# hsp-iit/roft

Measured on AMD Instinct MI355X. Metric: tracker frames/sec per object (640x480) + ADD-S vs CPU ref, higher is better.
Workload: dtype f64; 1 GPU; BASELINE config #4: 640x480, CV_32FC2 flow grid 1, 64 objects in total, 64 per GPU (sharded by object, no data-path collective; result rows all-gathered over RCCL at N > 1), masks+poses at 5 fps with 6-frame delay, flow-aided masks, re-sync and outlier rejection on, frames submitted in batches of at most 8; objects_per_gpu=64, objects_total=64, width=640, height=480, batch_frames=8, ranks=1, backend=nccl

## Files before the change

roft_amd/csrc/k_ukf.hip:

```cpp
#include "roft_device.h"

#pragma clang fp contract(fast)

namespace roft {

#ifdef ROFT_UKF_PROFILE
#define TICK(L, i) do { __syncthreads(); if (threadIdx.x == 0) { long long _t = clock64(); (L).dbg[i] += _t - (L).t0; (L).t0 = _t; } } while (0)
#else
#define TICK(L, i) do {} while (0)
#endif

constexpr int kUkfThreads = 256;

__device__ __forceinline__ void wave_sync()
{
    __builtin_amdgcn_fence(__ATOMIC_RELEASE, "wavefront");
    __builtin_amdgcn_wave_barrier();
    __builtin_amdgcn_fence(__ATOMIC_ACQUIRE, "wavefront");
}

__device__ __forceinline__ void quat_mul(const double a[4], const double b[4], double o[4])
{
    const double w = a[0] * b[0] - a[1] * b[1] - a[2] * b[2] - a[3] * b[3];
    const double x = a[0] * b[1] + a[1] * b[0] + a[2] * b[3] - a[3] * b[2];
    const double y = a[0] * b[2] - a[1] * b[3] + a[2] * b[0] + a[3] * b[1];
    const double z = a[0] * b[3] + a[1] * b[2] - a[2] * b[1] + a[3] * b[0];
    o[0] = w; o[1] = x; o[2] = y; o[3] = z;
}

__device__ __forceinline__ void half_angle(double n, double& sin_over_n, double& c)
{
    const double h = 0.5 * n;
    if (h < 0.25) {
        const double x = h * h;
        const double sinc = 1.0 + x * (-1.0 / 6.0 + x * (1.0 / 120.0 + x * (-1.0 / 5040.0 + x * (1.0 / 362880.0 +
                            x * (-1.0 / 39916800.0 + x * (1.0 / 6227020800.0))))));
        c = 1.0 + x * (-0.5 + x * (1.0 / 24.0 + x * (-1.0 / 720.0 + x * (1.0 / 40320.0 + x * (-1.0 / 3628800.0 +
            x * (1.0 / 479001600.0 + x * (-1.0 / 87178291200.0)))))));
        sin_over_n = 0.5 * sinc;
    } else {
        sin_over_n = sin(h) / n;
        c = cos(h);
    }
}

__device__ __forceinline__ void quat_boxplus(const double q[4], const double r[3], double o[4])
{
    const double n2 = r[0] * r[0] + r[1] * r[1] + r[2] * r[2];
    double s, c;
    if (n2 < 0.25) {
        const double x = 0.25 * n2;
        s = 0.5 * (1.0 + x * (-1.0 / 6.0 + x * (1.0 / 120.0 + x * (-1.0 / 5040.0 + x * (1.0 / 362880.0 +
                   x * (-1.0 / 39916800.0 + x * (1.0 / 6227020800.0)))))));
        c = 1.0 + x * (-0.5 + x * (1.0 / 24.0 + x * (-1.0 / 720.0 + x * (1.0 / 40320.0 + x * (-1.0 / 3628800.0 +
            x * (1.0 / 479001600.0 + x * (-1.0 / 87178291200.0)))))));
    } else {
        half_angle(sqrt(n2), s, c);
    }
    const double qr[4] = {c, s * r[0], s * r[1], s * r[2]};
    quat_mul(qr, q, o);
}

__device__ __forceinline__ double fast_rcp(double d);

__device__ __forceinline__ void quat_diff(const double a[4], const double b[4], double o[3])
{
    const double bc[4] = {b[0], -b[1], -b[2], -b[3]};
    double p[4];
    quat_mul(a, bc, p);
    const double n2 = p[1] * p[1] + p[2] * p[2] + p[3] * p[3];
    const double sgn = (p[0] < 0.0) ? -1.0 : 1.0;
    double k;
    const double ip0 = fast_rcp(fabs(p[0]));
    const double t2 = n2 * (ip0 * ip0);
    if (t2 <= 0.01) {
        const double at = 1.0 + t2 * (-1.0 / 3.0 + t2 * (1.0 / 5.0 + t2 * (-1.0 / 7.0 + t2 * (1.0 / 9.0 + t2 * (-1.0 / 11.0 +
                          t2 * (1.0 / 13.0 + t2 * (-1.0 / 15.0 + t2 * (1.0 / 17.0))))))));
        k = sgn * 2.0 * at * ip0;
    } else {
        const double n = sqrt(n2);
        if (n == 0.0) { o[0] = o[1] = o[2] = 0.0; return; }
        k = sgn * 2.0 * atan2(n, fabs(p[0])) / n;
    }
    o[0] = k * p[1]; o[1] = k * p[2]; o[2] = k * p[3];
}

constexpr int kCols = 50;

struct UkfTab {
    unsigned jtab[11 * 36 * 2];
    unsigned short tri12[78], tri6[26];
};
static_assert(sizeof(UkfTab) % 16 == 0, "copied in 16-byte words");
constexpr int kUkfTabWords = sizeof(UkfTab) / 16;

struct UkfLds {
    alignas(16) UkfTab tab;
    double P[144];
    double V[144];
    double wP[12];
    double S[144];
    double cs[2][6][2];
    double Q[100];
    double VQ[100];
    double wQ[10];
    double rc[12], rs[12];
    int rp[12], rq[12];
    double mean[13];
    double cov[144];
    double Y[13 * kCols];
    double D[12 * kCols];
    double X[12 * kCols];
    double ymean[13];
    double M4[16], V4[16], w4[4];
    double Py[144], Pxy[144], K[144], KPy[144];
    double aug[12 * 24];
    double innov[12], Kin[12];
    double par[24];
    double meas[13];
    double red[4];
    int flag;
    int twist_timeout;
    long long t0;
    long long dbg[32];
};

__device__ __forceinline__ double fast_rcp(double d)
{
    double x = __builtin_amdgcn_rcp(d);
    x = fma(fma(-d, x, 1.0), x, x);
    x = fma(fma(-d, x, 1.0), x, x);
    return x;
}

__device__ __forceinline__ double fast_rsqrt(double d)
{
    double y = __builtin_amdgcn_rsq(d);
    const double h = 0.5 * d;
    y = fma(y, fma(-h * y, y, 0.5), y);
    y = fma(y, fma(-h * y, y, 0.5), y);
    return y;
}

__device__ __forceinline__ void schur_rotation(double app, double aqq, double apq, double& c, double& s)
{
    const double a = aqq - app, b = 2.0 * apq;
    const int e = __builtin_amdgcn_frexp_exp(fmax(fabs(a), fabs(b)));
    const float af = fabsf((float)ldexp(a, -e)), bf = fabsf((float)ldexp(b, -e));
    const float h2 = af * af + bf * bf;
    const float hyp = h2 * __builtin_amdgcn_rsqf(h2);
    const float tf = bf * __builtin_amdgcn_rcpf(af + hyp);
    const double t = ((a >= 0.0) == (b >= 0.0) || a == 0.0) ? (double)tf : -(double)tf;
    const double x = fma(t, t, 1.0);
    double y = (double)__builtin_amdgcn_rsqf((float)x);
    const double hx = 0.5 * x;
    y = fma(y, fma(-hx * y, y, 0.5), y);
    y = fma(y, fma(-hx * y, y, 0.5), y);
    c = y;
    s = t * y;
}

#ifndef ROFT_JACOBI_TOL
#define ROFT_JACOBI_TOL 1e-6
#endif
constexpr double kJacobiTol = ROFT_JACOBI_TOL;

__host__ __device__ __forceinline__ constexpr void jacobi_pair(int n, int round, int i, int& p, int& q)
{
    if (i == 0) { p = n - 1; q = round; }
    else {
        p = round + i; if (p >= n - 1) p -= n - 1;
        q = round - i; if (q < 0) q += n - 1;
    }
    if (p > q) { const int t = p; p = q; q = t; }
}

__device__ __noinline__ void jacobi_wave(double* A, double* V, int n, UkfLds& L)
{
    const int lane = threadIdx.x;
    for (int i = lane; i < n * n; i += 64) V[i] = ((i / n) == (i % n)) ? 1.0 : 0.0;
    wave_sync();
    const int half = n / 2;
    const bool active = lane < half * half;
    const int ba = active ? lane / half : 0, bb = active ? lane % half : 0;
    for (int sweep = 0; sweep < 40; ++sweep) {
        double off = 0.0, dg = 0.0;
        for (int i = lane; i < n * n; i += 64) {
            const int r = i / n, cidx = i % n;
            const double v = A[i];
            if (r == cidx) dg += v * v; else if (r < cidx) off += v * v;
        }
        for (int o = 32; o > 0; o >>= 1) { off += __shfl_xor(off, o, 64); dg += __shfl_xor(dg, o, 64); }
        if (off <= kJacobiTol * kJacobiTol * dg || off == 0.0) break;
        for (int round = 0; round < n - 1; ++round) {
            int pa, qa, pb, qb;
            jacobi_pair(n, round, ba, pa, qa);
            jacobi_pair(n, round, bb, pb, qb);
            double a00 = 0, a01 = 0, a10 = 0, a11 = 0, v00 = 0, v01 = 0, v10 = 0, v11 = 0;
            if (active) {
                a00 = A[pa * n + pb]; a01 = A[pa * n + qb]; a10 = A[qa * n + pb]; a11 = A[qa * n + qb];
                v00 = V[pa * n + pb]; v01 = V[pa * n + qb]; v10 = V[qa * n + pb]; v11 = V[qa * n + qb];
            }
            double c = 1.0, s = 0.0;
            if (active && ba == bb && a01 != 0.0) schur_rotation(a00, a11, a01, c, s);
            const double ca = __shfl(c, ba * half + ba, 64), sa = __shfl(s, ba * half + ba, 64);
            const double cb = __shfl(c, bb * half + bb, 64), sb = __shfl(s, bb * half + bb, 64);
            if (active) {
                double b00 = cb * a00 - sb * a01, b01 = sb * a00 + cb * a01;
                double b10 = cb * a10 - sb * a11, b11 = sb * a10 + cb * a11;
                double c00 = ca * b00 - sa * b10, c10 = sa * b00 + ca * b10;
                double c01 = ca * b01 - sa * b11, c11 = sa * b01 + ca * b11;
                if (ba == bb) { c01 = c10 = 0.5 * (c01 + c10); }
                A[pa * n + pb] = c00; A[pa * n + qb] = c01; A[qa * n + pb] = c10; A[qa * n + qb] = c11;
                V[pa * n + pb] = cb * v00 - sb * v01; V[pa * n + qb] = sb * v00 + cb * v01;
                V[qa * n + pb] = cb * v10 - sb * v11; V[qa * n + qb] = sb * v10 + cb * v11;
            }
            wave_sync();
        }
    }
    wave_sync();
}

constexpr UkfTab make_ukf_tab()
{
    UkfTab t{};
    for (int i = 0; i < 11 * 36; ++i) {
        const int round = i / 36, l = i % 36;
        int pa = 0, qa = 0, pb = 0, qb = 0;
        jacobi_pair(12, round, l / 6, pa, qa);
        jacobi_pair(12, round, l % 6, pb, qb);
        t.jtab[2 * i] = (unsigned)(pa * 12 + pb) | ((unsigned)(pa * 12 + qb) << 16);
        t.jtab[2 * i + 1] = (unsigned)(qa * 12 + pb) | ((unsigned)(qa * 12 + qb) << 16);
    }
    int e = 0;
    for (int i = 0; i < 12; ++i)
        for (int j = i; j < 12; ++j) t.tri12[e++] = (unsigned short)((i << 8) | j);
    e = 0;
    for (int i = 0; i < 6; ++i)
        for (int j = i; j < 6; ++j) t.tri6[e++] = (unsigned short)((i << 8) | j);
    return t;
}
alignas(16) __device__ const UkfTab g_ukf_tab = make_ukf_tab();

__device__ __noinline__ void jacobi12(double* A, double* V, UkfLds& L)
{
    const int tid = threadIdx.x, wave = tid >> 6, lane = tid & 63;
    for (int i = tid; i < 144; i += kUkfThreads) V[i] = ((i / 12) == (i % 12)) ? 1.0 : 0.0;
    __syncthreads();
    const bool act = lane < 36 && wave < 2;
    const int ba = act ? lane / 6 : 0, bb = act ? lane % 6 : 0;
    double* M = (wave == 0) ? A : V;
    for (int sweep = 0; sweep < 40; ++sweep) {
        if (wave == 0) {
            double off = 0.0, dg = 0.0;
            for (int i = lane; i < 144; i += 64) {
                const int r = i / 12, cidx = i % 12;
                const double v = A[i];
                if (r == cidx) dg += v * v; else if (r < cidx) off += v * v;
            }
            for (int o = 32; o > 0; o >>= 1) { off += __shfl_xor(off, o, 64); dg += __shfl_xor(dg, o, 64); }
            if (lane == 0) L.flag = (off <= kJacobiTol * kJacobiTol * dg || off == 0.0) ? 1 : 0;
        }
        __syncthreads();
        if (L.flag) break;
#ifdef ROFT_UKF_PROFILE
        if (tid == 0) L.dbg[16] += 1;
#endif
        for (int round = 0; round < 11; ++round) {
            int o00 = 0, o01 = 0, o10 = 0, o11 = 0;
            double x00 = 0, x01 = 0, x10 = 0, x11 = 0;
            if (act) {
                const unsigned pkx = L.tab.jtab[2 * (round * 36 + lane)], pky = L.tab.jtab[2 * (round * 36 + lane) + 1];
                o00 = pkx & 0xFFFF; o01 = pkx >> 16; o10 = pky & 0xFFFF; o11 = pky >> 16;
                x00 = M[o00]; x01 = M[o01]; x10 = M[o10]; x11 = M[o11];
                if (wave == 0 && ba == bb) {
                    double c = 1.0, s = 0.0;
                    if (x01 != 0.0) schur_rotation(x00, x11, x01, c, s);
// ... 310 lines not shown
        if (tid < 144) {
            const int i = tid / 12, j = tid % 12;
            double s = 0.0;
            for (int k = 0; k < 12; ++k) s += L.cov[i * 12 + k] * V0[k * 12 + j];
            T[tid] = s;
        }
        __syncthreads();
        if (tid < 144) {
            const int r = tid / 12, c = tid % 12;
            const int i = r < c ? r : c, j = r < c ? c : r;
            double s = 0.0;
            for (int k = 0; k < 12; ++k) s += V0[k * 12 + i] * T[k * 12 + j];
            L.P[tid] = s;
        }
        __syncthreads();
        jacobi12(L.P, L.V, L);
        if (tid < 144) {
            const int i = tid / 12, j = tid % 12;
            double s = 0.0;
            for (int k = 0; k < 12; ++k) s += V0[i * 12 + k] * L.V[k * 12 + j];
            T[tid] = s;
        }
        Vfull = T;
    } else {
        if (tid < 144) L.P[tid] = L.cov[tid];
        __syncthreads();
        jacobi12(L.P, L.V, L);
    }
    double inv_ss = 0.0, m1 = 0.0;
    if (tid < 144) {
        const int i = tid / 12, j = tid % 12;
        const double si = sqrt(fabs(L.P[i * 13])), sj = sqrt(fabs(L.P[j * 13]));
        inv_ss = (si + sj > 0.0) ? fast_rcp(si + sj) : 0.0;
        if (i == j) m1 = si;
        else m1 = 0.5 * (L.P[i * 12 + j] + L.P[j * 12 + i]) * inv_ss;
        M[tid] = (i == j) ? 0.0 : m1;
    }
    __syncthreads();
    if (tid < 144) {
        const int i = tid / 12, j = tid % 12;
        double x1sq = 0.0;
        for (int k = 0; k < 12; ++k) x1sq += M[i * 12 + k] * M[k * 12 + j];
        m1 -= x1sq * inv_ss;
    }
    __syncthreads();
    if (tid < 144) M[tid] = m1;
    __syncthreads();
    if (tid < 144) {
        const int i = tid / 12, j = tid % 12;
        double acc = 0.0;
        for (int k = 0; k < 12; ++k) acc += Vfull[i * 12 + k] * M[k * 12 + j];
        L.S[tid] = acc;
        if (warm) warm[tid] = Vfull[tid];
    }
    if (tid < 12) L.wP[tid] = L.P[tid * 13];
    if (warm && tid == 0) *warm_age = use ? age + 1 : 1;
    __syncthreads();
}

__device__ __noinline__ bool cholesky_state_sqrt(UkfLds& L, bool for_correction, double T, double guard_rot, double guard_bil)
{
    if (!(guard_rot > 0.0)) return false;
    const double th = fmax(L.cov[9 * 13], fmax(L.cov[10 * 13], L.cov[11 * 13]));
    const double wv = fmax(L.cov[3 * 13], fmax(L.cov[4 * 13], L.cov[5 * 13]));
    const double xx = fmax(L.cov[6 * 13], fmax(L.cov[7 * 13], L.cov[8 * 13]));
    const int ok_corr = (int)(th <= guard_rot) & (int)(wv * xx <= guard_bil), ok_pred = (int)(th + T * T * wv <= guard_rot);
    const bool ok = __builtin_amdgcn_readfirstlane(for_correction ? ok_corr : ok_pred) != 0;
#ifdef ROFT_UKF_PROFILE
    if (threadIdx.x == 0 && for_correction) { L.dbg[20] = (long long)(th * 1e9); L.dbg[21] = (long long)(wv * 1e9); L.dbg[22] = (long long)(xx * 1e9); }
#endif
    if (!ok) return false;
    return cholesky_rows<12>(L.cov, L.S, L.rc, L);
}

__device__ void ukf_predict(UkfLds& L, const ObjParams& prm, double T, const UtTable& ut, double* warm,
                            int* warm_age, double chol_guard)
{
    const int lane = threadIdx.x;
    const int n = 21;
    const UtW& w = ut_lookup(ut, n);
    const double sc = w.sc;
    constexpr int kPredCols = 25;
    const double wm0 = w.wm0 + 18.0 * w.wi, wc0 = w.wc0 + 18.0 * w.wi;

    if (prm.q_override) {
        for (int i = lane; i < 100; i += kUkfThreads) L.Q[i] = 0.0;
        __syncthreads();
        for (int i = lane; i < 81; i += kUkfThreads) L.Q[(i / 9) * 10 + (i % 9)] = prm.q_override[i];
    } else if (lane >= 192 && lane < 195) {
        const int i = lane - 192;
        const double psd = L.par[3 + i];
        L.Q[i * 10 + i] = psd * T;
        L.Q[(6 + i) * 10 + (6 + i)] = psd * (T * T * T / 3.0);
        L.Q[i * 10 + (6 + i)] = L.Q[(6 + i) * 10 + i] = psd * (T * T / 2.0);
        L.Q[(3 + i) * 10 + (3 + i)] = L.par[i];
    }
    TICK(L, 1);
    if (!cholesky_state_sqrt(L, false, T, chol_guard, 0.0)) decompose_state_cov(L, warm, warm_age);
    TICK(L, 2);

    if (lane < kPredCols) {
        double d[12], dn[12];
        sigma_perturbation(lane, 0, sc, false, 0.0, L, d, dn);
        double v[3], wv[3], x[3], q[4];
        for (int i = 0; i < 3; ++i) {
            v[i] = L.mean[i] + d[i];
            wv[i] = L.mean[3 + i] + d[3 + i];
            x[i] = L.mean[6 + i] + d[6 + i];
        }
        quat_boxplus(L.mean + 9, d + 9, q);
        for (int i = 0; i < 3; ++i) {
            L.Y[i * kCols + lane] = v[i];
            L.Y[(3 + i) * kCols + lane] = wv[i];
            L.Y[(6 + i) * kCols + lane] = x[i] + v[i] * T;
        }
        const double norm_w = sqrt(wv[0] * wv[0] + wv[1] * wv[1] + wv[2] * wv[2]) + 2.220446049250313e-16;
        double s, c;
        half_angle(norm_w * T, s, c);
        s *= T;
        L.Y[9 * kCols + lane] = c * q[0] + s * (-wv[0] * q[1] - wv[1] * q[2] - wv[2] * q[3]);
        L.Y[10 * kCols + lane] = c * q[1] + s * (wv[0] * q[0] - wv[2] * q[2] + wv[1] * q[3]);
        L.Y[11 * kCols + lane] = c * q[2] + s * (wv[1] * q[0] + wv[2] * q[1] - wv[0] * q[3]);
        L.Y[12 * kCols + lane] = c * q[3] + s * (wv[2] * q[0] - wv[1] * q[1] + wv[0] * q[2]);
    }
    __syncthreads();

    TICK(L, 3);
    if (lane >= 64 && lane < 192) linear_means8(L.Y, 9, kPredCols, wm0, w.wi, lane - 64, L.ymean);
    double qm[4];
    quaternion_mean(L.Y, 9, kPredCols, wm0, w.wi, qm, L);
    TICK(L, 4);
    if (lane == 64)
        for (int i = 0; i < 4; ++i) L.ymean[9 + i] = qm[i];
    if (lane < kPredCols) {
        for (int i = 0; i < 9; ++i) L.D[i * kCols + lane] = L.Y[i * kCols + lane] - L.ymean[i];
        const double q[4] = {L.Y[9 * kCols + lane], L.Y[10 * kCols + lane], L.Y[11 * kCols + lane],
                             L.Y[12 * kCols + lane]};
        double dq[3];
        quat_diff(q, qm, dq);
        for (int i = 0; i < 3; ++i) L.D[(9 + i) * kCols + lane] = dq[i];
    }
    __syncthreads();
    if (lane < 192) {
        const int e = min(lane >> 1, 77), ij = L.tab.tri12[e], i = ij >> 8, j = ij & 0xFF;
        double v = weighted_dot_pair(L.D + i * kCols, L.D + j * kCols, kPredCols, wc0, w.wi, lane & 1);
        if (j < 9) v += L.Q[i * 10 + j];
        if (lane < 156) L.cov[(lane & 1) ? j * 12 + i : i * 12 + j] = v;
    }
    if (lane >= 192 && lane < 205) L.mean[lane - 192] = L.ymean[lane - 192];
    __syncthreads();
    TICK(L, 5);
}

__device__ int ukf_correct(UkfLds& L, int type, const UtTable& ut, PoseBelief* out)
{
    const int lane = threadIdx.x;
    if (type == ROFT_MEAS_NONE) {
        for (int i = lane; i < 144; i += kUkfThreads) out->cov[i] = L.cov[i];
        if (lane < 13) out->mean[lane] = L.mean[lane];
        return 1;
    }
    const bool has_vel = (type == ROFT_MEAS_VELOCITY || type == ROFT_MEAS_POSE_VELOCITY);
    const bool has_pose = (type == ROFT_MEAS_POSE || type == ROFT_MEAS_POSE_VELOCITY);
    const int r = (has_vel ? 6 : 0) + (has_pose ? 6 : 0);
    const int m = r;
    const int mtot = (has_vel ? 6 : 0) + (has_pose ? 7 : 0);
    const int nlin = mtot - (has_pose ? 4 : 0);
    const int n = 12 + r;
    const UtW& w = ut_lookup(ut, n);
    const double sc = w.sc;
    const int n_add = r - (has_pose ? 3 : 0);
    const int ncols = 25 + (has_pose ? 6 : 0);
    const double wm0 = w.wm0 + 2.0 * n_add * w.wi, wc0 = w.wc0 + 2.0 * n_add * w.wi;

    auto meas_at = [&](int k) -> double {
        return L.meas[has_vel ? k : 6 + k];
    };
    if (lane < ncols) {
        double d[12], dn[12];
        sigma_perturbation(min(lane, 24), 0, sc, false, 0.0, L, d, dn);
        double rv[3] = {0.0, 0.0, 0.0};
        if (lane >= 25) {
            const int k = (lane - 25) % 3;
            const double amp = (lane < 28) ? sc : -sc;
            const double v = amp * sqrt(fabs(L.par[21 + k]));
#pragma unroll
            for (int i = 0; i < 3; ++i) { if (i == k) rv[i] = v; }
#pragma unroll
            for (int i = 0; i < 12; ++i) d[i] = 0.0;
        }
#ifdef ROFT_UKF_PROFILE
        if (lane == 0) { long long _t = clock64(); L.dbg[24] += _t - L.t0; L.t0 = _t; }
#endif
        double v[3], wv[3], x[3], q[4];
        for (int i = 0; i < 3; ++i) {
            v[i] = L.mean[i] + d[i];
            wv[i] = L.mean[3 + i] + d[3 + i];
            x[i] = L.mean[6 + i] + d[6 + i];
        }
        quat_boxplus(L.mean + 9, d + 9, q);
        for (int i = 0; i < 9; ++i) L.X[i * kCols + lane] = d[i];
        if (d[9] * d[9] + d[10] * d[10] + d[11] * d[11] < 9.0) {
            for (int i = 9; i < 12; ++i) L.X[i * kCols + lane] = d[i];
        } else {
            double dq[3];
            quat_diff(q, L.mean + 9, dq);
            for (int i = 0; i < 3; ++i) L.X[(9 + i) * kCols + lane] = dq[i];
        }

        int row = 0;
        if (has_vel) {
            const double p[3] = {-x[0], -x[1], -x[2]};
            const double cr[3] = {wv[1] * p[2] - wv[2] * p[1], wv[2] * p[0] - wv[0] * p[2], wv[0] * p[1] - wv[1] * p[0]};
            for (int i = 0; i < 3; ++i) {
                L.Y[(row + i) * kCols + lane] = v[i] + cr[i];
                L.Y[(row + 3 + i) * kCols + lane] = wv[i];
            }
            row += 6;
        }
        if (has_pose) {
            for (int i = 0; i < 3; ++i) L.Y[(row + i) * kCols + lane] = x[i];
            double qo[4];
            quat_boxplus(q, rv, qo);
            for (int i = 0; i < 4; ++i) L.Y[(row + 3 + i) * kCols + lane] = qo[i];
        }
    }
    __syncthreads();

    TICK(L, 8);
    if (lane >= 64 && lane < 192) linear_means8(L.Y, nlin, ncols, wm0, w.wi, lane - 64, L.ymean);
    double qm[4] = {1.0, 0.0, 0.0, 0.0};
    if (has_pose) {
        quaternion_mean(L.Y, nlin, ncols, wm0, w.wi, qm, L);
        if (lane == 64)
            for (int i = 0; i < 4; ++i) L.ymean[nlin + i] = qm[i];
    } else {
        __syncthreads();
    }
    TICK(L, 23);
    if (lane < ncols) {
        for (int i = 0; i < nlin; ++i) L.D[i * kCols + lane] = L.Y[i * kCols + lane] - L.ymean[i];
        if (has_pose) {
            const double q[4] = {L.Y[nlin * kCols + lane], L.Y[(nlin + 1) * kCols + lane],
                                 L.Y[(nlin + 2) * kCols + lane], L.Y[(nlin + 3) * kCols + lane]};
            double dq[3];
            quat_diff(q, qm, dq);
            for (int i = 0; i < 3; ++i) L.D[(nlin + i) * kCols + lane] = dq[i];
        }
    }
    if (lane >= 224 && lane < 224 + nlin) L.innov[lane - 224] = -(L.ymean[lane - 224] - meas_at(lane - 224));
    if (has_pose && lane == 255) {
        const double mq[4] = {meas_at(nlin), meas_at(nlin + 1), meas_at(nlin + 2), meas_at(nlin + 3)};
        double dq[3];
        quat_diff(mq, qm, dq);
        for (int i = 0; i < 3; ++i) L.innov[nlin + i] = dq[i];
    }
    __syncthreads();
    TICK(L, 9);
    const int r_base = has_vel ? 12 : 18;
    if (m == 6) {
        if (lane < 192) {
            const int e = min(lane >> 1, 92);
            const double *ar, *br;
            int o0, o1 = -1;
            double add = 0.0;
            if (e < 72) { ar = L.X + (e / 6) * kCols; br = L.D + (e % 6) * kCols; o0 = e; }
            else {
                const int ij = L.tab.tri6[e - 72], i = ij >> 8, j = ij & 0xFF;
                ar = L.D + i * kCols; br = L.D + j * kCols; o0 = i * 6 + j; o1 = j * 6 + i;
                if (i == j && i < n_add) add = fabs(L.par[r_base + i]);
            }
            const double v = weighted_dot_pair(ar, br, ncols, wc0, w.wi, lane & 1) + add;
            if (lane < 186) {
                if (e < 72) { if (!(lane & 1)) L.Pxy[o0] = v; }
                else L.Py[(lane & 1) ? o1 : o0] = v;
            }
        }
    } else {
        const int nxy = 12 * m, ntri = m * (m + 1) / 2;
        if (lane < nxy) {
            const int i = lane / m, j = lane % m;
            L.Pxy[lane] = weighted_dot(L.X + i * kCols, L.D + j * kCols, ncols, wc0, w.wi);
        } else if (lane - nxy < ntri) {
            int u = lane - nxy, i = 0;
            while (u >= m - i) { u -= m - i; ++i; }
            const int j = i + u;
            double sum = weighted_dot(L.D + i * kCols, L.D + j * kCols, ncols, wc0, w.wi);
            if (i == j && i < n_add) sum += fabs(L.par[r_base + i]);
            L.Py[i * m + j] = sum;
            L.Py[j * m + i] = sum;
        }
    }
    __syncthreads();

    TICK(L, 10);
    if (!((m == 6) ? cholesky_rows<6>(L.Py, L.aug, L.rc, L) : cholesky_rows<12>(L.Py, L.aug, L.rc, L))) {
        for (int i = lane; i < 144; i += kUkfThreads) out->cov[i] = L.cov[i];
        if (lane < 13) out->mean[lane] = L.mean[lane];
        return 2;
    }
    TICK(L, 11);
    if (m == 6) chol_solve_rows<6>(L.aug, L.rc, L.Pxy, L.K);
    else chol_solve_rows<12>(L.aug, L.rc, L.Pxy, L.K);
    __syncthreads();
    TICK(L, 25);
    if (lane < 12 * m) {
        const int i = lane / m, j = lane % m;
        double s = 0.0;
        for (int k = 0; k < m; ++k) s += L.K[i * m + k] * L.Py[k * m + j];
        L.KPy[i * m + j] = s;
    } else if (lane >= 192 && lane < 192 + 12) {
        const int i = lane - 192;
        double s = 0.0;
        for (int k = 0; k < m; ++k) s += L.K[i * m + k] * L.innov[k];
        L.Kin[i] = s;
    }
    __syncthreads();
    TICK(L, 26);
    if (lane < 144) {
        const int i = lane / 12, j = lane % 12;
        double s = 0.0;
        for (int k = 0; k < m; ++k) s += L.KPy[i * m + k] * L.K[j * m + k];
        out->cov[lane] = L.cov[lane] - s;
    } else if (lane >= 192 && lane < 192 + 9) {
        out->mean[lane - 192] = L.mean[lane - 192] + L.Kin[lane - 192];
    } else if (lane == 192 + 9) {
        double qo[4];
        quat_boxplus(L.mean + 9, L.Kin + 9, qo);
        for (int i = 0; i < 4; ++i) out->mean[9 + i] = qo[i];
    }
    __syncthreads();
    TICK(L, 12);
    return 0;
}

__device__ bool ukf_one_step(const EngineArrays& a, const FrameCtrl& c, int obj, int step, const UtTable& ut, UkfLds& L)
{
    ObjState& st = a.state[obj];
    struct {
        int op, src, do_predict, n_corr, type0, type1, dst0, dst1, twist_slot;
    } sd;
    {
        const StepDesc& d = c.steps[step];
        sd.op = d.op; sd.src = d.src; sd.do_predict = d.do_predict; sd.n_corr = d.n_corr;
        sd.type0 = d.type[0]; sd.type1 = d.type[1]; sd.dst0 = d.dst[0]; sd.dst1 = d.dst[1]; sd.twist_slot = d.twist_slot;
    }
    if (!sd.op) return true;
    const ObjParams& prm = a.params[obj];
    const int lane = threadIdx.x;
    const int lin = c.lane, cur = c.cur_slot;

#ifdef ROFT_UKF_PROFILE
    if (lane < 32) L.dbg[lane] = 0;
    if (lane == 0) L.t0 = clock64();
    __syncthreads();
#endif
    const PoseBelief& src = st.belief[sd.src];
    for (int i = lane; i < 144; i += kUkfThreads) L.cov[i] = src.cov[i];
    if (lane < 13) L.mean[lane] = src.mean[lane];
    static_assert(offsetof(ObjParams, R_q) == 21 * sizeof(double), "L.par mirrors the head of ObjParams");
    if (lane >= 160 && lane < 184) L.par[lane - 160] = reinterpret_cast<const double*>(&prm)[lane - 160];
    if (lane >= 192) {
        const int i = lane - 192;
        if (a.handoff) {
            const int want = c.frame_idx - ((c.frame_idx - sd.twist_slot) & (kTwistRing - 1)) + 1;
            if (lane == 192) {
                const long long t0 = wall_clock64();
                unsigned spins = 0;
                int timed_out = 0;
                while (__hip_atomic_load(&st.twist_tag[sd.twist_slot], __ATOMIC_RELAXED, __HIP_MEMORY_SCOPE_AGENT) < want) {
                    __builtin_amdgcn_s_sleep(1);
                    if ((++spins & 4095u) == 0u && wall_clock64() - t0 > 200000000ll) {
                        if (a.dev_error) __hip_atomic_store(a.dev_error, ROFT_DEV_ERROR_TWIST_WAIT, __ATOMIC_RELAXED, __HIP_MEMORY_SCOPE_SYSTEM);
                        timed_out = 1;
                        break;
                    }
                }
                L.twist_timeout = timed_out;
            }
            __atomic_signal_fence(__ATOMIC_SEQ_CST);
            if (i < 6) L.meas[i] = __longlong_as_double((long long)__hip_atomic_load(
                reinterpret_cast<const unsigned long long*>(&st.twist_hist[sd.twist_slot][i]), __ATOMIC_RELAXED, __HIP_MEMORY_SCOPE_AGENT));
        } else if (i < 6) {
            L.meas[i] = st.twist_hist[sd.twist_slot][i];
        }
        if (i >= 6 && i < 13) L.meas[i] = (i < 9) ? c.pose_x[i - 6] : c.pose_q[i - 9];
    }
    __syncthreads();
    if (a.handoff && L.twist_timeout) return false;

    TICK(L, 0);
    if (sd.do_predict) {
        ukf_predict(L, prm, c.dt, ut, st.warm_V[cur][0], &st.warm_age[cur][0], a.ukf_chol_guard);
        PoseBelief& pr = st.belief[B_PRED + lin];
        for (int i = lane; i < 144; i += kUkfThreads) pr.cov[i] = L.cov[i];
        if (lane < 13) pr.mean[lane] = L.mean[lane];
    }
    if (sd.n_corr == 0) {
        PoseBelief& d = st.belief[sd.dst0];
        for (int i = lane; i < 144; i += kUkfThreads) d.cov[i] = L.cov[i];
        if (lane < 13) d.mean[lane] = L.mean[lane];
        if (roft_object_output* row = log_row(a, c, obj))
            if (lane < 13 && sd.dst0 == cur) row->pose[lane] = L.mean[lane];
        return true;
    }
    TICK(L, 6);
    if (!cholesky_state_sqrt(L, true, c.dt, a.ukf_chol_guard, a.ukf_chol_guard_bil))
        decompose_state_cov(L, st.warm_V[cur][1], &st.warm_age[cur][1]);
    TICK(L, 7);
    int status = 0;
    for (int k = 0; k < sd.n_corr; ++k) {
        const int rc = ukf_correct(L, k == 0 ? sd.type0 : sd.type1, ut, &st.belief[k == 0 ? sd.dst0 : sd.dst1]);
        status |= rc << (4 * k);
        __syncthreads();
    }
    if (lane == 0) st.lane[lin].ukf_status = status;
    if (roft_object_output* row = log_row(a, c, obj)) {
        __syncthreads();
        if (lane < 13) row->pose[lane] = st.belief[cur].mean[lane];
    }
#ifdef ROFT_UKF_PROFILE
    __syncthreads();
    if (lane < 32) st.dbg[lane] = L.dbg[lane];
#endif
    return true;
}

#ifndef PRIO_UKF
#define PRIO_UKF 3
#endif
#ifdef UKF_WAVES_PER_EU
__attribute__((amdgpu_waves_per_eu(UKF_WAVES_PER_EU, UKF_WAVES_PER_EU)))
#endif
__global__ __launch_bounds__(kUkfThreads) void ukf_chain_kernel(EngineArrays a, UtTable ut, int first_segment, int lin)
{
    ROFT_RESIDENT(a, RK_UKF_CHAIN);
    __shared__ UkfLds L;
    uint4 tab_word = make_uint4(0u, 0u, 0u, 0u);
    if ((int)threadIdx.x < kUkfTabWords) tab_word = reinterpret_cast<const uint4*>(&g_ukf_tab)[threadIdx.x];
    __builtin_amdgcn_s_setprio(PRIO_UKF);
#ifdef ROFT_UKF_WALL
    const long long w_entry = wall_clock64();
    __shared__ unsigned s_ticket;
    if (threadIdx.x == 0) {
        s_ticket = atomicAdd(reinterpret_cast<unsigned*>(&a.state[0].dbg[30 + 0]) + lin, 1u);
        long long* rec = a.state[(s_ticket / a.n_obj) % a.n_obj].dbg + lin * 8;
        const long long now = wall_clock64();
        atomicMax(reinterpret_cast<unsigned long long*>(&rec[0]), (unsigned long long)((1ll << 62) - now));
        atomicMax(reinterpret_cast<unsigned long long*>(&rec[1]), (unsigned long long)now);
    }
    __syncthreads();
#endif
    const int obj = blockIdx.x;
    ObjState& st = a.state[obj];
    PoseLane& pl = st.lane[lin];
    int t = first_segment ? 0 : pl.pc_frame, step = first_segment ? 0 : pl.pc_step;
    if (t >= a.T) return;
    const int vote_lane = threadIdx.x & 63;
    const unsigned mine = (unsigned)__ballot(vote_lane < a.T && frame_ctrl(a, vote_lane, obj).lane == lin);
    if ((mine >> t) == 0u) {
        if (threadIdx.x == 0) { pl.pending_frame = -1; pl.pc_frame = a.T; pl.pc_step = 0; }
        return;
    }
    if (!first_segment && pl.pending_frame >= 0) {
        const FrameCtrl& pc = frame_ctrl(a, pl.pending_frame, obj);
        double Lk[2];
        for (int k = 0; k < 2; ++k) {
            long long hi = 0, lo = 0;
            double n2 = 0.0;
            for (int p = 0; p < pl.n_parts[k]; ++p) { hi += pl.part_hi[k][p]; lo += pl.part_lo[k][p]; n2 += pl.part_cnt[k][p]; }
            const double e = LikelihoodSum::value(hi, lo);
            Lk[k] = (n2 == 0.0) ? 1.7976931348623157e308 : (e / n2) / 1.0;
            if (threadIdx.x == 0) { pl.outlier_L[k] = Lk[k]; pl.outlier_cnt[k] = n2; }
        }
        const double L0 = Lk[0], L1 = Lk[1];
        const int sel = (L0 > 2.0 * L1) ? 1 : 0;
        const PoseBelief& src = st.belief[b_alt(lin, sel)];
        PoseBelief& dst = st.belief[pc.cur_slot];
        for (int i = threadIdx.x; i < 144; i += kUkfThreads) dst.cov[i] = src.cov[i];
        if (threadIdx.x < 13) dst.mean[threadIdx.x] = src.mean[threadIdx.x];
        roft_object_output* row = log_row(a, pc, obj);
        if (row && threadIdx.x < 13) row->pose[threadIdx.x] = src.mean[threadIdx.x];
        if (threadIdx.x == 0) {
            pl.outlier_selected = sel;
            if (row) { row->outlier_selected = sel; row->outlier_L[0] = L0; row->outlier_L[1] = L1; }
        }
        __syncthreads();
    }
    static_assert(kUkfTabWords <= kUkfThreads, "one 16-byte word of the tables per thread");
    if ((int)threadIdx.x < kUkfTabWords) reinterpret_cast<uint4*>(&L.tab)[threadIdx.x] = tab_word;
    for (int i = threadIdx.x; i < 100; i += kUkfThreads) L.Q[i] = 0.0;
    __syncthreads();
    bool pending = false;
    __shared__ FrameCtrl s_c;
    int staged = -1;
#ifdef ROFT_UKF_WALL
    const long long w_t0 = wall_clock64();
    int w_steps = 0;
    long long* w_rec = a.state[(s_ticket / a.n_obj) % a.n_obj].dbg + lin * 8;
#endif
    while (t < a.T) {
        if (!((mine >> t) & 1u)) { ++t; step = 0; continue; }
        if (staged != t) {
            __syncthreads();
            stage_ctrl(&s_c, frame_ctrl(a, t, obj));
            staged = t;
            __syncthreads();
        }
        const FrameCtrl& c = s_c;
        if (step == 0 && threadIdx.x == 0) {
            pl.outlier_selected = -1;
            if (roft_object_output* row0 = log_row(a, c, obj)) row0->outlier_selected = -1;
        }
        if (step >= c.n_steps) { ++t; step = 0; continue; }
#ifdef ROFT_UKF_WALL
        const long long w_s0 = wall_clock64();
#endif
        if (c.steps[step].op && !ukf_one_step(a, c, obj, step, ut, L)) {
            __syncthreads();
            t = a.T;
            step = 0;
            pending = false;
            break;
        }
#ifdef ROFT_UKF_WALL
        if (threadIdx.x == 0 && w_steps == 0) {
            atomicAdd(reinterpret_cast<unsigned long long*>(&st.dbg[26]), (unsigned long long)(w_s0 - w_entry));
            atomicAdd(reinterpret_cast<unsigned long long*>(&st.dbg[27]), (unsigned long long)(wall_clock64() - w_s0));
            atomicAdd(reinterpret_cast<unsigned long long*>(&st.dbg[19]), 1ull);
        }
        if (threadIdx.x == 0 && w_steps > 0) {
            const long long d = wall_clock64() - w_s0;
            const int bin = d < 1800 ? 0 : (d < 2200 ? 1 : (d < 3000 ? 2 : 3));
            atomicAdd(reinterpret_cast<unsigned long long*>(&st.dbg[20 + bin]), 1ull);
            if (bin == 3) atomicAdd(reinterpret_cast<unsigned long long*>(&st.dbg[24]), (unsigned long long)d);
            if (bin == 3) atomicAdd(reinterpret_cast<unsigned long long*>(&st.dbg[25]), (unsigned long long)(c.steps[step].n_corr * 100 + c.steps[step].type[0]));
        }
        ++w_steps;
#endif
        __syncthreads();
        pending = (step == c.outlier_step);
        ++step;
        if (pending) break;
    }
#ifdef ROFT_UKF_WALL
    if (threadIdx.x == 0) {
        const long long w_t1 = wall_clock64();
        atomicAdd(reinterpret_cast<unsigned long long*>(&st.dbg[28]), (unsigned long long)(w_t1 - w_t0));
        atomicAdd(reinterpret_cast<unsigned long long*>(&st.dbg[29]), (unsigned long long)w_steps);
        atomicMax(reinterpret_cast<unsigned long long*>(&w_rec[2]), (unsigned long long)w_t1);
        atomicMax(reinterpret_cast<unsigned long long*>(&w_rec[3]), (unsigned long long)w_steps);
        atomicAdd(reinterpret_cast<unsigned long long*>(&w_rec[4]), (unsigned long long)w_steps);
        atomicAdd(reinterpret_cast<unsigned long long*>(&w_rec[5]), 1ull);
        if (w_steps > 0) atomicMax(reinterpret_cast<unsigned long long*>(&w_rec[6]), (unsigned long long)((w_t1 - w_t0) / w_steps));
        if (w_steps > 0) atomicMax(reinterpret_cast<unsigned long long*>(&w_rec[7]), (unsigned long long)(w_t1 - w_t0));
    }
#endif
    if (threadIdx.x == 0) {
        pl.pending_frame = pending ? t : -1;
        pl.pc_frame = t;
        pl.pc_step = step;
    }
}

void launch_ukf_chain(const EngineArrays& a, roft_ut_params ut, bool first_segment, int lin, hipStream_t s, hipEvent_t stop)
{
    UtTable tab;
    for (int k = 0; k < 3; ++k) tab.w[k] = ut_weights(18 + 3 * k, ut);
    hipExtLaunchKernelGGL(ukf_chain_kernel, dim3(a.n_obj), dim3(kUkfThreads), 0, s, nullptr, stop, 0, a, tab,
                          first_segment ? 1 : 0, lin);
}

}
```

Baseline: 1.708 million object-frames/s.

## Carry UKF belief in LDS across steps and prefetch next step's control and measurements

Keeps the corrected mean and covariance in shared memory so the next step can skip reloading its source belief from global memory when the slot matches. The fourth wavefront prefetches the next frame's control block into a double-buffered shared FrameCtrl and the next step's twist and pose measurements into a double-buffered meas array, overlapping that with predict. The outlier resolution path now preloads both alternative beliefs in registers and seeds the LDS carry. This removes global round trips and barriers per step, at the cost of more LDS and complex key and slot bookkeeping that could go stale under handoff.

After: 1.678 million object-frames/s. 0.982x the previous value.

```diff
diff --git a/roft_amd/csrc/k_ukf.hip b/roft_amd/csrc/k_ukf.hip
--- a/roft_amd/csrc/k_ukf.hip
+++ b/roft_amd/csrc/k_ukf.hip
@@ -117,12 +117,19 @@
     double aug[12 * 24];
     double innov[12], Kin[12];
     double par[24];
-    double meas[13];
+    double meas[2][13];
+    int pf_key[2];
     double red[4];
     int flag;
     int twist_timeout;
     long long t0;
+    long long prof_ctrl;
     long long dbg[32];
+};
+
+struct StepCarry {
+    int slot;
+    int mb;
 };
 
 __device__ __forceinline__ double fast_rcp(double d)
@@ -739,7 +746,7 @@
     TICK(L, 5);
 }
 
-__device__ int ukf_correct(UkfLds& L, int type, const UtTable& ut, PoseBelief* out)
+__device__ int ukf_correct(UkfLds& L, int type, const UtTable& ut, PoseBelief* out, const double* meas, bool keep)
 {
     const int lane = threadIdx.x;
     if (type == ROFT_MEAS_NONE) {
@@ -761,7 +768,7 @@
     const double wm0 = w.wm0 + 2.0 * n_add * w.wi, wc0 = w.wc0 + 2.0 * n_add * w.wi;
 
     auto meas_at = [&](int k) -> double {
-        return L.meas[has_vel ? k : 6 + k];
+        return meas[has_vel ? k : 6 + k];
     };
     if (lane < ncols) {
         double d[12], dn[12];
@@ -908,20 +915,27 @@
         const int i = lane / 12, j = lane % 12;
         double s = 0.0;
         for (int k = 0; k < m; ++k) s += L.KPy[i * m + k] * L.K[j * m + k];
-        out->cov[lane] = L.cov[lane] - s;
+        const double v = L.cov[lane] - s;
+        out->cov[lane] = v;
+        if (keep) L.cov[lane] = v;
     } else if (lane >= 192 && lane < 192 + 9) {
-        out->mean[lane - 192] = L.mean[lane - 192] + L.Kin[lane - 192];
+        const double v = L.mean[lane - 192] + L.Kin[lane - 192];
+        out->mean[lane - 192] = v;
+        if (keep) L.mean[lane - 192] = v;
     } else if (lane == 192 + 9) {
         double qo[4];
         quat_boxplus(L.mean + 9, L.Kin + 9, qo);
         for (int i = 0; i < 4; ++i) out->mean[9 + i] = qo[i];
+        if (keep)
+            for (int i = 0; i < 4; ++i) L.mean[9 + i] = qo[i];
     }
     __syncthreads();
     TICK(L, 12);
     return 0;
 }
 
-__device__ bool ukf_one_step(const EngineArrays& a, const FrameCtrl& c, int obj, int step, const UtTable& ut, UkfLds& L)
+__device__ bool ukf_one_step(const EngineArrays& a, const FrameCtrl& c, FrameCtrl* nc, int obj, int t, int step, int t_next,
+                             int stage_next, const UtTable& ut, UkfLds& L, StepCarry& cy)
 {
     ObjState& st = a.state[obj];
     struct {
@@ -937,18 +951,29 @@
     const int lane = threadIdx.x;
     const int lin = c.lane, cur = c.cur_slot;
 
+    const int wave3 = lane >= 192, i3 = lane - 192;
+    const int src_slot = __builtin_amdgcn_readfirstlane(sd.src);
+    const int key = (t << 8) | step;
+    const bool carried = src_slot == cy.slot;
+    const bool fetched = __builtin_amdgcn_readfirstlane(L.pf_key[cy.mb ^ 1]) == key;
+    if (fetched) cy.mb ^= 1;
+    double* const meas = L.meas[cy.mb];
 #ifdef ROFT_UKF_PROFILE
     if (lane < 32) L.dbg[lane] = 0;
     if (lane == 0) L.t0 = clock64();
     __syncthreads();
-#endif
-    const PoseBelief& src = st.belief[sd.src];
-    for (int i = lane; i < 144; i += kUkfThreads) L.cov[i] = src.cov[i];
-    if (lane < 13) L.mean[lane] = src.mean[lane];
-    static_assert(offsetof(ObjParams, R_q) == 21 * sizeof(double), "L.par mirrors the head of ObjParams");
-    if (lane >= 160 && lane < 184) L.par[lane - 160] = reinterpret_cast<const double*>(&prm)[lane - 160];
-    if (lane >= 192) {
-        const int i = lane - 192;
+    if (lane == 0) { L.dbg[27] = L.prof_ctrl; L.prof_ctrl = 0; }
+#endif
+    if (!carried) {
+        const PoseBelief& src = st.belief[src_slot];
+        for (int i = lane; i < 144; i += kUkfThreads) L.cov[i] = src.cov[i];
+        if (lane < 13) L.mean[lane] = src.mean[lane];
+#ifdef ROFT_UKF_PROFILE
+        if (lane == 0) { __builtin_amdgcn_s_waitcnt(0); L.dbg[28] = clock64() - L.t0; }
+#endif
+    }
+    if (!fetched && wave3) {
+        const int i = i3;
         if (a.handoff) {
             const int want = c.frame_idx - ((c.frame_idx - sd.twist_slot) & (kTwistRing - 1)) + 1;
             if (lane == 192) {
@@ -966,22 +991,64 @@
                 L.twist_timeout = timed_out;
             }
             __atomic_signal_fence(__ATOMIC_SEQ_CST);
-            if (i < 6) L.meas[i] = __longlong_as_double((long long)__hip_atomic_load(
+            if (i < 6) meas[i] = __longlong_as_double((long long)__hip_atomic_load(
                 reinterpret_cast<const unsigned long long*>(&st.twist_hist[sd.twist_slot][i]), __ATOMIC_RELAXED, __HIP_MEMORY_SCOPE_AGENT));
         } else if (i < 6) {
-            L.meas[i] = st.twist_hist[sd.twist_slot][i];
-        }
-        if (i >= 6 && i < 13) L.meas[i] = (i < 9) ? c.pose_x[i - 6] : c.pose_q[i - 9];
-    }
-    __syncthreads();
-    if (a.handoff && L.twist_timeout) return false;
+            meas[i] = st.twist_hist[sd.twist_slot][i];
+        }
+        if (i >= 6 && i < 13) meas[i] = (i < 9) ? c.pose_x[i - 6] : c.pose_q[i - 9];
+#ifdef ROFT_UKF_PROFILE
+        if (lane == 192) { __builtin_amdgcn_s_waitcnt(0); L.dbg[29] = clock64() - L.t0; }
+#endif
+    }
+    if (!carried || !fetched) {
+        __syncthreads();
+        if (!fetched && a.handoff && L.twist_timeout) return false;
+    }
 
     TICK(L, 0);
+    if (stage_next >= 0 && wave3) {
+        constexpr int n16 = (int)(sizeof(FrameCtrl) / 16);
+        const uint4* g = reinterpret_cast<const uint4*>(&frame_ctrl(a, stage_next, obj));
+        for (int i = i3; i < n16; i += 64) reinterpret_cast<uint4*>(nc)[i] = g[i];
+    }
     if (sd.do_predict) {
         ukf_predict(L, prm, c.dt, ut, st.warm_V[cur][0], &st.warm_age[cur][0], a.ukf_chol_guard);
         PoseBelief& pr = st.belief[B_PRED + lin];
         for (int i = lane; i < 144; i += kUkfThreads) pr.cov[i] = L.cov[i];
         if (lane < 13) pr.mean[lane] = L.mean[lane];
+    }
+    if (wave3) {
+        wave_sync();
+        const int c_steps = __builtin_amdgcn_readfirstlane(c.n_steps), c_out = __builtin_amdgcn_readfirstlane(c.outlier_step);
+        const FrameCtrl* nf = nullptr;
+        int ns = 0, nt = t;
+        if (step != c_out) {
+            if (step + 1 < c_steps) { nf = &c; ns = step + 1; }
+            else if (t_next >= 0 && __builtin_amdgcn_readfirstlane(nc->n_steps) > 0) { nf = nc; nt = t_next; }
+        }
+        if (nf && __builtin_amdgcn_readfirstlane(nf->steps[ns].op)) {
+            double* const nm = L.meas[cy.mb ^ 1];
+            const int slot = __builtin_amdgcn_readfirstlane(nf->steps[ns].twist_slot);
+            int have = 1;
+            if (a.handoff) {
+                const int fidx = __builtin_amdgcn_readfirstlane(nf->frame_idx);
+                const int want = fidx - ((fidx - slot) & (kTwistRing - 1)) + 1;
+                have = __builtin_amdgcn_readfirstlane(
+                           __hip_atomic_load(&st.twist_tag[slot], __ATOMIC_RELAXED, __HIP_MEMORY_SCOPE_AGENT)) >= want;
+                if (have) {
+                    __atomic_signal_fence(__ATOMIC_SEQ_CST);
+                    if (i3 < 6) nm[i3] = __longlong_as_double((long long)__hip_atomic_load(
+                        reinterpret_cast<const unsigned long long*>(&st.twist_hist[slot][i3]), __ATOMIC_RELAXED, __HIP_MEMORY_SCOPE_AGENT));
+                }
+            } else if (i3 < 6) {
+                nm[i3] = st.twist_hist[slot][i3];
+            }
+            if (have) {
+                if (i3 >= 6 && i3 < 13) nm[i3] = (i3 < 9) ? nf->pose_x[i3 - 6] : nf->pose_q[i3 - 9];
+                if (i3 == 0) L.pf_key[cy.mb ^ 1] = (nt << 8) | ns;
+            }
+        }
     }
     if (sd.n_corr == 0) {
         PoseBelief& d = st.belief[sd.dst0];
@@ -989,6 +1056,7 @@
         if (lane < 13) d.mean[lane] = L.mean[lane];
         if (roft_object_output* row = log_row(a, c, obj))
             if (lane < 13 && sd.dst0 == cur) row->pose[lane] = L.mean[lane];
+        cy.slot = __builtin_amdgcn_readfirstlane(sd.dst0);
         return true;
     }
     TICK(L, 6);
@@ -997,14 +1065,21 @@
     TICK(L, 7);
     int status = 0;
     for (int k = 0; k < sd.n_corr; ++k) {
-        const int rc = ukf_correct(L, k == 0 ? sd.type0 : sd.type1, ut, &st.belief[k == 0 ? sd.dst0 : sd.dst1]);
+        const int rc = ukf_correct(L, k == 0 ? sd.type0 : sd.type1, ut, &st.belief[k == 0 ? sd.dst0 : sd.dst1], meas,
+                                   k == sd.n_corr - 1);
         status |= rc << (4 * k);
         __syncthreads();
     }
+    const int last_dst = __builtin_amdgcn_readfirstlane(sd.n_corr == 1 ? sd.dst0 : sd.dst1);
+    cy.slot = last_dst;
     if (lane == 0) st.lane[lin].ukf_status = status;
     if (roft_object_output* row = log_row(a, c, obj)) {
-        __syncthreads();
-        if (lane < 13) row->pose[lane] = st.belief[cur].mean[lane];
+        if (last_dst == __builtin_amdgcn_readfirstlane(cur)) {
+            if (lane < 13) row->pose[lane] = L.mean[lane];
+        } else {
+            __syncthreads();
+            if (lane < 13) row->pose[lane] = st.belief[cur].mean[lane];
+        }
     }
 #ifdef ROFT_UKF_PROFILE
     __syncthreads();
@@ -1049,38 +1124,61 @@
         if (threadIdx.x == 0) { pl.pending_frame = -1; pl.pc_frame = a.T; pl.pc_step = 0; }
         return;
     }
+    int carry_slot = -1;
     if (!first_segment && pl.pending_frame >= 0) {
         const FrameCtrl& pc = frame_ctrl(a, pl.pending_frame, obj);
+        const int tid = threadIdx.x;
+        const int cur_slot = pc.cur_slot;
+        int n_parts[2];
+        long long p_hi[2][kMaxOutlierParts], p_lo[2][kMaxOutlierParts];
+        double p_cnt[2][kMaxOutlierParts];
+        double alt_cov[2] = {0.0, 0.0}, alt_mean[2] = {0.0, 0.0};
+#pragma unroll
+        for (int k = 0; k < 2; ++k) {
+            n_parts[k] = pl.n_parts[k];
+#pragma unroll
+            for (int p = 0; p < kMaxOutlierParts; ++p) { p_hi[k][p] = pl.part_hi[k][p]; p_lo[k][p] = pl.part_lo[k][p]; p_cnt[k][p] = pl.part_cnt[k][p]; }
+            const PoseBelief& alt = st.belief[b_alt(lin, k)];
+            if (tid < 144) alt_cov[k] = alt.cov[tid];
+            if (tid < 13) alt_mean[k] = alt.mean[tid];
+        }
         double Lk[2];
+#pragma unroll
         for (int k = 0; k < 2; ++k) {
             long long hi = 0, lo = 0;
             double n2 = 0.0;
-            for (int p = 0; p < pl.n_parts[k]; ++p) { hi += pl.part_hi[k][p]; lo += pl.part_lo[k][p]; n2 += pl.part_cnt[k][p]; }
+#pragma unroll
+            for (int p = 0; p < kMaxOutlierParts; ++p)
+                if (p < n_parts[k]) { hi += p_hi[k][p]; lo += p_lo[k][p]; n2 += p_cnt[k][p]; }
             const double e = LikelihoodSum::value(hi, lo);
             Lk[k] = (n2 == 0.0) ? 1.7976931348623157e308 : (e / n2) / 1.0;
-            if (threadIdx.x == 0) { pl.outlier_L[k] = Lk[k]; pl.outlier_cnt[k] = n2; }
+            if (tid == 0) { pl.outlier_L[k] = Lk[k]; pl.outlier_cnt[k] = n2; }
         }
         const double L0 = Lk[0], L1 = Lk[1];
         const int sel = (L0 > 2.0 * L1) ? 1 : 0;
-        const PoseBelief& src = st.belief[b_alt(lin, sel)];
-        PoseBelief& dst = st.belief[pc.cur_slot];
-        for (int i = threadIdx.x; i < 144; i += kUkfThreads) dst.cov[i] = src.cov[i];
-        if (threadIdx.x < 13) dst.mean[threadIdx.x] = src.mean[threadIdx.x];
+        PoseBelief& dst = st.belief[cur_slot];
+        const double cv = sel ? alt_cov[1] : alt_cov[0], mv = sel ? alt_mean[1] : alt_mean[0];
+        if (tid < 144) { dst.cov[tid] = cv; L.cov[tid] = cv; }
+        if (tid < 13) { dst.mean[tid] = mv; L.mean[tid] = mv; }
         roft_object_output* row = log_row(a, pc, obj);
-        if (row && threadIdx.x < 13) row->pose[threadIdx.x] = src.mean[threadIdx.x];
-        if (threadIdx.x == 0) {
+        if (row && tid < 13) row->pose[tid] = mv;
+        if (tid == 0) {
             pl.outlier_selected = sel;
             if (row) { row->outlier_selected = sel; row->outlier_L[0] = L0; row->outlier_L[1] = L1; }
         }
-        __syncthreads();
+        carry_slot = cur_slot;
     }
     static_assert(kUkfTabWords <= kUkfThreads, "one 16-byte word of the tables per thread");
     if ((int)threadIdx.x < kUkfTabWords) reinterpret_cast<uint4*>(&L.tab)[threadIdx.x] = tab_word;
     for (int i = threadIdx.x; i < 100; i += kUkfThreads) L.Q[i] = 0.0;
+    static_assert(offsetof(ObjParams, R_q) == 21 * sizeof(double), "L.par mirrors the head of ObjParams");
+    if (threadIdx.x >= 160 && threadIdx.x < 184) L.par[threadIdx.x - 160] = reinterpret_cast<const double*>(&a.params[obj])[threadIdx.x - 160];
+    if (threadIdx.x == 0) { L.pf_key[0] = L.pf_key[1] = -1; L.twist_timeout = 0; L.prof_ctrl = 0; }
     __syncthreads();
     bool pending = false;
-    __shared__ FrameCtrl s_c;
-    int staged = -1;
+    __shared__ FrameCtrl s_c[2];
+    int cb = 0, staged = -1, staged_next = -1, c_n_steps = 0, c_outlier = -1;
+    StepCarry cy = {__builtin_amdgcn_readfirstlane(carry_slot), 0};
 #ifdef ROFT_UKF_WALL
     const long long w_t0 = wall_clock64();
     int w_steps = 0;
@@ -1089,21 +1187,41 @@
     while (t < a.T) {
         if (!((mine >> t) & 1u)) { ++t; step = 0; continue; }
         if (staged != t) {
-            __syncthreads();
-            stage_ctrl(&s_c, frame_ctrl(a, t, obj));
+            if (staged_next == t) {
+                cb ^= 1;
+#ifdef ROFT_UKF_PROFILE
+                if (threadIdx.x == 0) L.prof_ctrl = 0;
+#endif
+            } else {
+#ifdef ROFT_UKF_PROFILE
+                const long long p0 = clock64();
+#endif
+                __syncthreads();
+                stage_ctrl(&s_c[cb], frame_ctrl(a, t, obj));
+                __syncthreads();
+#ifdef ROFT_UKF_PROFILE
+                if (threadIdx.x == 0) L.prof_ctrl = clock64() - p0;
+#endif
+            }
             staged = t;
-            __syncthreads();
-        }
-        const FrameCtrl& c = s_c;
+            staged_next = -1;
+            c_n_steps = __builtin_amdgcn_readfirstlane(s_c[cb].n_steps);
+            c_outlier = __builtin_amdgcn_readfirstlane(s_c[cb].outlier_step);
+        }
+        const FrameCtrl& c = s_c[cb];
         if (step == 0 && threadIdx.x == 0) {
             pl.outlier_selected = -1;
             if (roft_object_output* row0 = log_row(a, c, obj)) row0->outlier_selected = -1;
         }
-        if (step >= c.n_steps) { ++t; step = 0; continue; }
+        if (step >= c_n_steps) { ++t; step = 0; continue; }
+        const unsigned later = (t + 1 < 32) ? (mine >> (t + 1)) : 0u;
+        const int t_next = later ? t + 1 + __builtin_ctz(later) : -1;
+        const int stage_next = (t_next >= 0 && staged_next != t_next) ? t_next : -1;
 #ifdef ROFT_UKF_WALL
         const long long w_s0 = wall_clock64();
 #endif
-        if (c.steps[step].op && !ukf_one_step(a, c, obj, step, ut, L)) {
+        const bool op = __builtin_amdgcn_readfirstlane(c.steps[step].op) != 0;
+        if (op && !ukf_one_step(a, c, &s_c[cb ^ 1], obj, t, step, t_next, stage_next, ut, L, cy)) {
             __syncthreads();
             t = a.T;
             step = 0;
@@ -1125,8 +1243,9 @@
         }
         ++w_steps;
 #endif
+        if (op && stage_next >= 0) staged_next = t_next;
         __syncthreads();
-        pending = (step == c.outlier_step);
+        pending = (step == c_outlier);
         ++step;
         if (pending) break;
     }
```
